# dkarpushkin/rs-pathtracing

Hardware: AMD Instinct MI355X
Metric: Msamples/sec cornell_box 1920x1080x256spp at 1/2/4/8 MI355X; RMS pixel delta (higher is better)
Workload: dtype f64; 1 GPU; cornell_box.json 1920x1080 256spp depth 8; config=c2, width=1920, height=1080, spp=256, depth=8, seed=1, parallelism=single GPU, wf_slots=2

## Files before the change

### rs-pathtracing_amd/csrc/pt_accel.cpp

```cpp
#include "pt_accel.hpp"

#include <algorithm>
#include <cmath>
#include <cstdlib>
#include <cstring>
#include <stdexcept>

namespace pt {

DBox shape_box(const HostShape &s) {
    double lo[3], hi[3];
    switch (s.type) {
    case RECTANGLE:
        lo[0] = s.x0; lo[1] = s.y0; lo[2] = -0.0001;
        hi[0] = s.x1; hi[1] = s.y1; hi[2] = 0.0001;
        break;
    case MARCH:
        if (s.func == 0) {
            lo[0] = -1.45; lo[1] = -(1.45 / 2.05); lo[2] = -1.45;
            hi[0] = 1.45; hi[1] = 1.45 / 2.05; hi[2] = 1.45;
        } else {
            const double r = std::fabs(s.fr);
            lo[0] = lo[1] = lo[2] = -r;
            hi[0] = hi[1] = hi[2] = r;
        }
        break;
    case TORUS: {
        const double a = s.radius + s.tube_radius;
        lo[0] = -a; lo[1] = -a; lo[2] = -s.tube_radius;
        hi[0] = a; hi[1] = a; hi[2] = s.tube_radius;
        break;
    }
    default:
        lo[0] = lo[1] = lo[2] = -1.0;
        hi[0] = hi[1] = hi[2] = 1.0;
    }
    DBox b;
    for (int k = 0; k < 3; k++) {
        b.lo[k] = INFINITY;
        b.hi[k] = -INFINITY;
    }
    for (int i = 0; i < 2; i++)
        for (int j = 0; j < 2; j++)
            for (int k = 0; k < 2; k++) {
                double p[3] = {i ? hi[0] : lo[0], j ? hi[1] : lo[1], k ? hi[2] : lo[2]};
                for (int r = 0; r < 3; r++) {
                    double v = p[0] * s.direct[r][0] + p[1] * s.direct[r][1] + p[2] * s.direct[r][2] + s.direct[r][3];
                    b.lo[r] = std::min(b.lo[r], v);
                    b.hi[r] = std::max(b.hi[r], v);
                }
            }
    double extent = 0;
    for (int r = 0; r < 3; r++)
        extent = std::max({extent, std::fabs(b.lo[r]), std::fabs(b.hi[r]), b.hi[r] - b.lo[r]});
    double pad = 1e-7 * extent + 1e-9;
    if (s.type == MARCH) pad += 2.0 * std::fabs(s.step);
    for (int r = 0; r < 3; r++) {
        b.lo[r] -= pad;
        b.hi[r] += pad;
    }
    return b;
}

namespace {

struct Builder {
    const std::vector<DBox> &boxes;
    Accel &out;
    int leaf_max = 1;
    struct TNode {
        DNode n;
        int axis, left, right;
    };
    std::vector<TNode> tree;

    void thread(int t, int oct, size_t base) {
        const size_t me = out.nodes.size();
        out.nodes.push_back(tree[t].n);
        if (tree[t].left >= 0) {
            const bool neg = (oct >> tree[t].axis) & 1;
            thread(neg ? tree[t].right : tree[t].left, oct, base);
            thread(neg ? tree[t].left : tree[t].right, oct, base);
        }
        out.nodes[me].skip = (int32_t)(out.nodes.size() - base);
    }

    int emit(std::vector<int32_t> &ids, size_t a, size_t b) {
        const int me = (int)tree.size();
        tree.push_back(TNode{DNode{}, 0, -1, -1});
        DNode n{};
        for (int k = 0; k < 3; k++) {
            n.lo[k] = INFINITY;
            n.hi[k] = -INFINITY;
        }
        double clo[3] = {INFINITY, INFINITY, INFINITY}, chi[3] = {-INFINITY, -INFINITY, -INFINITY};
        for (size_t i = a; i < b; i++) {
            const DBox &x = boxes[ids[i]];
            for (int k = 0; k < 3; k++) {
                n.lo[k] = std::min(n.lo[k], x.lo[k]);
                n.hi[k] = std::max(n.hi[k], x.hi[k]);
                double c = 0.5 * (x.lo[k] + x.hi[k]);
                clo[k] = std::min(clo[k], c);
                chi[k] = std::max(chi[k], c);
            }
        }
        if (b - a <= (size_t)leaf_max) {
            n.first = (int32_t)out.leaf.size();
            n.count = (int32_t)(b - a);
            for (size_t i = a; i < b; i++) out.leaf.push_back(ids[i]);
            tree[me].n = n;
            return me;
        }
        int axis = 0;
        for (int k = 1; k < 3; k++)
            if (chi[k] - clo[k] > chi[axis] - clo[axis]) axis = k;
        if (b - a > 2) {
            constexpr int NB = 32;
            auto area = [](const double *lo, const double *hi) {
                const double x = hi[0] - lo[0], y = hi[1] - lo[1], z = hi[2] - lo[2];
                return x * y + y * z + z * x;
            };
            double best = INFINITY;
            int bk = -1, bi = -1;
            for (int k = 0; k < 3; k++) {
                const double ext = chi[k] - clo[k];
                if (!(ext > 0.0)) continue;
                int cnt[NB] = {};
                double blo[NB][3], bhi[NB][3];
                for (int j = 0; j < NB; j++)
                    for (int r = 0; r < 3; r++) blo[j][r] = INFINITY, bhi[j][r] = -INFINITY;
                for (size_t i = a; i < b; i++) {
                    const DBox &x = boxes[ids[i]];
                    int j = (int)((0.5 * (x.lo[k] + x.hi[k]) - clo[k]) / ext * NB);
                    j = j < 0 ? 0 : (j >= NB ? NB - 1 : j);
                    cnt[j]++;
                    for (int r = 0; r < 3; r++) blo[j][r] = std::min(blo[j][r], x.lo[r]), bhi[j][r] = std::max(bhi[j][r], x.hi[r]);
                }
                double rlo[NB][3], rhi[NB][3];
                int rc[NB];
                for (int j = NB - 1; j >= 0; j--) {
                    for (int r = 0; r < 3; r++) {
                        rlo[j][r] = j + 1 < NB ? std::min(rlo[j + 1][r], blo[j][r]) : blo[j][r];
                        rhi[j][r] = j + 1 < NB ? std::max(rhi[j + 1][r], bhi[j][r]) : bhi[j][r];
                    }
                    rc[j] = (j + 1 < NB ? rc[j + 1] : 0) + cnt[j];
                }
                double llo[3] = {INFINITY, INFINITY, INFINITY}, lhi[3] = {-INFINITY, -INFINITY, -INFINITY};
                int lc = 0;
                for (int j = 0; j + 1 < NB; j++) {
                    lc += cnt[j];
                    for (int r = 0; r < 3; r++) llo[r] = std::min(llo[r], blo[j][r]), lhi[r] = std::max(lhi[r], bhi[j][r]);
                    if (lc == 0 || rc[j + 1] == 0) continue;
                    const double c = lc * area(llo, lhi) + rc[j + 1] * area(rlo[j + 1], rhi[j + 1]);
                    if (c < best) best = c, bk = k, bi = j;
                }
            }
            if (bk >= 0) {
                const double ext = chi[bk] - clo[bk];
                auto left = [&](int32_t id) {
                    const DBox &x = boxes[id];
                    int j = (int)((0.5 * (x.lo[bk] + x.hi[bk]) - clo[bk]) / ext * NB);
                    j = j < 0 ? 0 : (j >= NB ? NB - 1 : j);
                    return j <= bi;
                };
                const size_t m = (size_t)(std::stable_partition(ids.begin() + a, ids.begin() + b, left) - ids.begin());
                if (m > a && m < b) {
                    const int l = emit(ids, a, m);
                    const int r = emit(ids, m, b);
                    n.count = 0;
                    n.first = 0;
                    tree[me] = TNode{n, bk, l, r};
                    return me;
                }
            }
        }
        size_t mid = a + (b - a) / 2;
        std::nth_element(ids.begin() + a, ids.begin() + mid, ids.begin() + b, [&](int32_t x, int32_t y) {
            double cx = boxes[x].lo[axis] + boxes[x].hi[axis], cy = boxes[y].lo[axis] + boxes[y].hi[axis];
            return cx < cy || (cx == cy && x < y);
        });
        const int l = emit(ids, a, mid);
        const int r = emit(ids, mid, b);
        n.count = 0;
        n.first = 0;
        tree[me] = TNode{n, axis, l, r};
        return me;
    }
};

}

static bool make_grid(Accel &a) {
    double lo[3], hi[3];
    for (int k = 0; k < 3; k++) lo[k] = INFINITY, hi[k] = -INFINITY;
    for (const DNode &n : a.nodes)
        for (int k = 0; k < 3; k++) lo[k] = std::min(lo[k], n.lo[k]), hi[k] = std::max(hi[k], n.hi[k]);
    for (int k = 0; k < 3; k++) {
        if (!(std::isfinite(lo[k]) && std::isfinite(hi[k]) && std::isfinite(hi[k] - lo[k]))) return false;
        double step = std::ldexp(1.0, std::ilogb(std::max(hi[k] - lo[k], 1e-300) / 65535.0));
        for (int guard = 0;; guard++) {
            const double g0 = std::floor(lo[k] / step) * step;
            if (std::isfinite(g0) && std::ceil((hi[k] - g0) / step) <= 65535.0 && g0 <= lo[k]) {
                a.qg0[k] = g0;
                a.qgs[k] = step;
                break;
            }
            step *= 2.0;
            if (!std::isfinite(step) || guard > 64) return false;
        }
    }
    return true;
}
static double q_down(const Accel &a, double v, int k) {
    double q = std::floor((v - a.qg0[k]) / a.qgs[k]);
    while (q > 0 && a.qg0[k] + q * a.qgs[k] > v) q -= 1.0;
    return std::max(0.0, std::min(65535.0, q));
}
static double q_up(const Accel &a, double v, int k) {
    double q = std::ceil((v - a.qg0[k]) / a.qgs[k]);
    while (q < 65535.0 && a.qg0[k] + q * a.qgs[k] < v) q += 1.0;
    return std::max(0.0, std::min(65535.0, q));
}

void build_qnodes(Accel &a, const Scene &sc) {
    const size_t per_oct = a.nodes.size() / BVH_OCTANTS;
    if (!make_grid(a)) return;
    std::vector<DNodeQ> out;
    out.reserve(a.nodes.size());
    std::vector<int32_t> rec_of(a.leaf.size() + 1, -1);
    std::vector<DLeafRec> recs;
    for (size_t ni = 0; ni < per_oct; ni++) {
        const DNode &n = a.nodes[ni];
        if (n.count != 1 || !(a.cnodes[ni].first_count >> 31)) continue;
        const int id = a.leaf[n.first];
        const DShape d = to_device(sc.shapes[id]);
        DLeafRec l{};
        l.m[0] = d.inv[0], l.m[1] = d.inv[5], l.m[2] = d.inv[10];
        l.m[3] = d.inv[3], l.m[4] = d.inv[7], l.m[5] = d.inv[11];
        l.shape = id;
        l.axis = d.axis;
        rec_of[n.first] = (int32_t)recs.size();
        recs.push_back(l);
    }
    double bound = 0.0;
    for (int k = 0; k < 3; k++) bound = std::max(bound, std::fabs(a.qg0[k]));
    for (size_t ni = 0; ni < a.nodes.size(); ni++) {
        const DNode &n = a.nodes[ni];
        const int oct = (int)(ni / per_oct);
        DNodeQ c{};
        for (int k = 0; k < 3; k++) {
            const double ql = q_down(a, n.lo[k], k), qh = q_up(a, n.hi[k], k);
            if (a.qg0[k] + ql * a.qgs[k] > n.lo[k] || a.qg0[k] + qh * a.qgs[k] < n.hi[k]) return;
            bound = std::max({bound, std::fabs(a.qg0[k] + ql * a.qgs[k]), std::fabs(a.qg0[k] + qh * a.qgs[k])});
            const bool neg = (oct >> k) & 1;
            c.q[k] = (uint16_t)(neg ? qh : ql);
            c.q[3 + k] = (uint16_t)(neg ? ql : qh);
        }
        if (n.count == 0) {
            if (n.skip < 0) return;
            c.link = (uint32_t)n.skip;
        } else {
            if ((size_t)n.skip != ni % per_oct + 1 || n.count > 63) return;
            const uint32_t fc = a.cnodes[ni].first_count;
            const bool direct = fc >> 31;
            uint32_t first = fc & 0xffffffu;
            if (direct) {
                if (rec_of[n.first] < 0) return;
                first = (uint32_t)rec_of[n.first];
            }
            c.link = 1u << 31 | (direct ? 1u << 30 : 0u) | (uint32_t)n.count << 24 | first;
        }
        out.push_back(c);
    }
    a.qnodes.swap(out);
    a.qleaves.swap(recs);
    a.qbound = (float)bound;
    if ((double)a.qbound < bound) a.qbound = std::nextafter(a.qbound, INFINITY);
}

std::vector<DQGrid> pack_qnodes(const Accel &a) {
    if (a.qnodes.empty()) return {};
    const size_t ro = qleaf_offset(a.nodes_per_octant()), rb = a.qleaves.size() * sizeof(DLeafRec);
    std::vector<DQGrid> buf((ro + rb) / sizeof(DQGrid));
    for (int k = 0; k < 3; k++) buf[0].g0[k] = a.qg0[k], buf[0].gs[k] = a.qgs[k];
    buf[0].bound = a.qbound;
    std::memcpy(&buf[1], a.qnodes.data(), a.qnodes.size() * sizeof(DNodeQ));
    if (rb) std::memcpy((char *)buf.data() + ro, a.qleaves.data(), rb);
    return buf;
}

Accel build_accel(const Scene &sc, int json_shapes, int leaf_max) {
    Accel a;
    a.boxes.reserve(sc.shapes.size());
    for (auto &s : sc.shapes) a.boxes.push_back(shape_box(s));
    std::vector<int32_t> rest;
    bool small = json_shapes <= LIN_MAX;
    for (int32_t i = 0; i < (int32_t)sc.shapes.size(); i++) {
        if (sc.shapes[i].type == MARCH) a.march.push_back(i);
        else if ((small && i < json_shapes) || sc.shapes[i].type == TORUS) a.lin.push_back(i);
        else rest.push_back(i);
    }
    if (rest.size() > 64) {
        auto ext = [&](int32_t i) {
            const DBox &b = a.boxes[i];
            return std::max({b.hi[0] - b.lo[0], b.hi[1] - b.lo[1], b.hi[2] - b.lo[2]});
        };
        std::vector<double> e;
        e.reserve(rest.size());
        for (int32_t i : rest) e.push_back(ext(i));
        std::nth_element(e.begin(), e.begin() + e.size() / 2, e.end());
        const double big = 64.0 * e[e.size() / 2];
        std::vector<int32_t> keep;
        keep.reserve(rest.size());
        for (int32_t i : rest) {
            if (ext(i) > big && a.lin.size() < (size_t)LIN_MAX) a.lin.push_back(i);
            else keep.push_back(i);
        }
        rest.swap(keep);
    }
    if (!rest.empty()) {
        Builder b{a.boxes, a};
        b.leaf_max = std::max(1, std::min(16, leaf_max));
        const int root = b.emit(rest, 0, rest.size());
        a.nodes.reserve(b.tree.size() * BVH_OCTANTS);
        for (int oct = 0; oct < BVH_OCTANTS; oct++) b.thread(root, oct, a.nodes.size());
    }
    a.cnodes.reserve(a.nodes.size());
    const size_t per_oct = a.nodes.size() / BVH_OCTANTS;
    for (size_t ni = 0; ni < a.nodes.size(); ni++) {
        const DNode &n = a.nodes[ni];
        const int oct = per_oct ? (int)(ni / per_oct) : 0;
        if (n.first < 0 || n.first >= (1 << 24) || n.count < 0 || n.count > 255)
            throw std::runtime_error("BVH too large for the compact node form (leaf index >= 2^24)");
        DNodeC c{};
        for (int k = 0; k < 3; k++) {
            float lo = (float)n.lo[k], hi = (float)n.hi[k];
            if ((double)lo > n.lo[k]) lo = std::nextafter(lo, -INFINITY);
            if ((double)hi < n.hi[k]) hi = std::nextafter(hi, INFINITY);
            const bool neg = (oct >> k) & 1;
            c.nr[k] = neg ? hi : lo;
            c.fr[k] = neg ? lo : hi;
        }
        c.skip = n.skip;
        for (int k = 0; k < 3; k++) a.bvh_bound = std::max({a.bvh_bound, std::fabs(c.nr[k]), std::fabs(c.fr[k])});
        if (n.count == 1 && a.leaf[n.first] >= 0 && a.leaf[n.first] < (1 << 24))
            c.first_count = (uint32_t)a.leaf[n.first] | 1u << 24 | 1u << 31;
        else
            c.first_count = (uint32_t)n.first | (uint32_t)n.count << 24;
        a.cnodes.push_back(c);
    }
    if (per_oct >= (size_t)BIG_BVH_NODES) {
        build_qnodes(a, sc);
    }
    return a;
}

}
```

### rs-pathtracing_amd/csrc/pt_accel.hpp

```cpp
#pragma once
#include <array>
#include <cstdint>
#include <vector>

#include "pt_scene.hpp"
#include "pt_types.hpp"

namespace pt {

constexpr int BVH_OCTANTS = 8;
struct Accel {
    std::vector<DNode> nodes;
    std::vector<DNodeC> cnodes;
    int nodes_per_octant() const { return (int)(nodes.size() / BVH_OCTANTS); }
    std::vector<int32_t> leaf;
    std::vector<int32_t> lin;
    std::vector<int32_t> march;
    std::vector<DBox> boxes;
    float bvh_bound = 0.f;
    std::vector<DNodeQ> qnodes;
    std::vector<DLeafRec> qleaves;
    double qg0[3] = {0, 0, 0}, qgs[3] = {0, 0, 0};
    float qbound = 0.f;
};

constexpr int LIN_MAX = 32;

Accel build_accel(const Scene &sc, int json_shapes, int leaf_max = 1);
void build_qnodes(Accel &a, const Scene &sc);

std::vector<DQGrid> pack_qnodes(const Accel &a);
static_assert(sizeof(DLeafRec) % sizeof(DQGrid) == 0, "pack_qnodes sizes its buffer in DQGrid units");

static_assert(sizeof(dev::Scene) == 136, "a new dev::Scene field must be set by view_set_scene or view_set_accel");
inline void view_set_scene(dev::Scene &v, const Scene &sc, const DShape *shapes, const DMaterial *mats,
                           const DTexture *tex, const DPerlin *perlin, const DImage *images, const uint8_t *pixels) {
    v.shapes = shapes;
    v.mats = mats;
    v.tex = tex;
    v.perlin = perlin;
    v.images = images;
    v.pixels = pixels;
    v.nmats = (int)sc.materials.size();
    v.ext = scene_builds(sc).ext;
}
inline void view_set_accel(dev::Scene &v, const DNodeC *nodes, const DQGrid *qnodes, const int32_t *leaf,
                           const int32_t *lin, const int32_t *march, const DBox *boxes, int nnodes, int nlin,
                           int nmarch, float bvh_bound) {
    v.nodes = nodes;
    v.qnodes = qnodes;
    v.leaf = leaf;
    v.lin = lin;
    v.march = march;
    v.boxes = boxes;
    v.nnodes = nnodes;
    v.nlin = nlin;
    v.nmarch = nmarch;
    v.bvh_bound = bvh_bound;
}
inline void view_set_accel(dev::Scene &v, const Accel &a, const DNodeC *nodes, const DQGrid *qnodes,
                           const int32_t *leaf, const int32_t *lin, const int32_t *march, const DBox *boxes) {
    view_set_accel(v, nodes, qnodes, leaf, lin, march, boxes, a.nodes_per_octant(), (int)a.lin.size(),
                   (int)a.march.size(), a.bvh_bound);
}
inline void view_set_accel(dev::Scene &v, const dev::Scene &a) {
    view_set_accel(v, a.nodes, a.qnodes, a.leaf, a.lin, a.march, a.boxes, a.nnodes, a.nlin, a.nmarch, a.bvh_bound);
}
constexpr size_t VIEW_ACCEL_BUFS = 6;
inline std::array<const void *, 13> view_buffers(const dev::Scene &v) {
    return {v.nodes, v.qnodes, v.leaf,   v.lin,    v.march,  v.boxes, v.shapes,
            v.mats,  v.tex,    v.perlin, v.images, v.pixels, v.guard};
}
inline void view_of_host(dev::Scene &v, const Scene &sc, const Accel &a, const std::vector<DShape> &shapes,
                         const std::vector<DMaterial> &mats, const std::vector<DQGrid> &qbuf) {
    auto ptr = [](const auto &vec) { return vec.empty() ? nullptr : vec.data(); };
    view_set_scene(v, sc, ptr(shapes), ptr(mats), ptr(sc.textures), ptr(sc.perlins), ptr(sc.images), ptr(sc.pixels));
    view_set_accel(v, a, ptr(a.cnodes), ptr(qbuf), ptr(a.leaf), ptr(a.lin), ptr(a.march), ptr(a.boxes));
}

DBox shape_box(const HostShape &s);

}
```

### rs-pathtracing_amd/csrc/pt_device.hpp

```cpp
#pragma once
#include <hip/hip_runtime.h>

#include <cstdint>

#include "pt_lprof.hpp"
#include "pt_march.hpp"
#include "pt_torus.hpp"
#include "pt_types.hpp"

namespace pt {
namespace dev {

__device__ __forceinline__ bool stopped(const int *flag) {
    return flag && __hip_atomic_load(flag, __ATOMIC_RELAXED, __HIP_MEMORY_SCOPE_SYSTEM) != 0;
}

struct V3 {
    double x, y, z;
};
PT_HD V3 v3(double x, double y, double z) { return V3{x, y, z}; }
PT_HD V3 add(V3 a, V3 b) { return v3(a.x + b.x, a.y + b.y, a.z + b.z); }
PT_HD V3 sub(V3 a, V3 b) { return v3(a.x - b.x, a.y - b.y, a.z - b.z); }
PT_HD double dot(V3 a, V3 b) { return a.x * b.x + a.y * b.y + a.z * b.z; }
PT_HD V3 scale(V3 a, double s) { return v3(a.x * s, a.y * s, a.z * s); }
// ... 1 lines not shown
PT_HD V3 neg(V3 a) { return v3(-a.x, -a.y, -a.z); }
PT_HD V3 normalize(V3 a) { return divs(a, sqrt(dot(a, a))); }
PT_HD bool approx_zero(double a) { return fabs(a - 0.0) < 1e-15; }

constexpr uint64_t GAMMA = 0x9E3779B97F4A7C15ull;
PT_HD uint64_t mix64(uint64_t z) {
    z = (z ^ (z >> 30)) * 0xBF58476D1CE4E5B9ull;
    z = (z ^ (z >> 27)) * 0x94D049BB133111EBull;
    return z ^ (z >> 31);
}
PT_HD uint64_t sample_key(uint64_t seed, uint64_t pixel, uint64_t sample) {
    uint64_t k = mix64(seed ^ 0x6A09E667F3BCC909ull);
    k = mix64(k + (pixel + 1) * GAMMA);
    return mix64(k + (sample + 1) * 0xD1B54A32D192ED03ull);
}
PT_HD double bits_to_double(uint64_t b) {
    union {
        uint64_t u;
        double d;
    } x;
    x.u = b;
    return x.d;
}
struct Rng {
    uint64_t s;
    PT_HD uint64_t next() {
        s += GAMMA;
        return mix64(s);
    }
    PT_HD double gen() { return (double)(next() >> 11) * (1.0 / 9007199254740992.0); }
    PT_HD double uniform(double lo, double sc) {
        double v = bits_to_double((next() >> 12) | (1023ull << 52));
        return (v - 1.0) * sc + lo;
    }
};

PT_HD V3 xf_point(const double *m, V3 p) {
    return v3(p.x * m[0] + p.y * m[1] + p.z * m[2] + m[3], p.x * m[4] + p.y * m[5] + p.z * m[6] + m[7],
              p.x * m[8] + p.y * m[9] + p.z * m[10] + m[11]);
}
PT_HD V3 xf_vector(const double *m, V3 v) {
    return v3(v.x * m[0] + v.y * m[1] + v.z * m[2], v.x * m[4] + v.y * m[5] + v.z * m[6],
              v.x * m[8] + v.y * m[9] + v.z * m[10]);
}
PT_HD V3 xf_normal(const double *m, V3 n) {
    return v3(n.x * m[0] + n.y * m[4] + n.z * m[8], n.x * m[1] + n.y * m[5] + n.z * m[9],
              n.x * m[2] + n.y * m[6] + n.z * m[10]);
}



PT_HD bool sphere_t(V3 o, V3 d, double min_t, double max_t, double *t) {
    double a = dot(d, d);
    double hb = dot(d, o);
    double c = dot(o, o) - 1.0;
    double disc = hb * hb - a * c;
    if (disc < 0.0) return false;
    double x;
    if (disc == 0.0) {
        x = -hb * a;
    } else {
        double sq = sqrt(disc);
        x = (-hb - sq) / a;
        if (x < min_t || x > max_t) {
            x = (-hb + sq) / a;
            if (x < min_t || x > max_t) return false;
        }
    }
    *t = x;
    return true;
}
PT_HD bool axis_ray_ok(const V3 &o, const V3 &d) {
    const double sum = o.x + o.y + o.z + d.x + d.y + d.z;
    return sum - sum == 0.0 && fabs(d.x) > 1e-200 && fabs(d.y) > 1e-200 && fabs(d.z) > 1e-200;
}
PT_HD bool sphere_axis_t(const double *m, V3 ro, V3 rd, double min_t, double max_t, double *t) {
    const V3 o = v3(ro.x * m[0] + m[3], ro.y * m[5] + m[7], ro.z * m[10] + m[11]);
    const V3 d = v3(rd.x * m[0], rd.y * m[5], rd.z * m[10]);
    return sphere_t(o, d, min_t, max_t, t);
}
PT_HD bool rect_t(const double *p, V3 o, V3 d, double min_t, double max_t, double *t) {
    double tt = -o.z / d.z;
    if (tt < min_t || tt > max_t) return false;
    double px = o.x + d.x * tt, py = o.y + d.y * tt;
    if (px < p[0] || px > p[2] || py < p[1] || py > p[3]) return false;
    *t = tt;
    return true;
}
PT_HD bool cube_t(V3 o, V3 d, double min_t, double max_t, double *t) {
    double lx = (-1.0 - o.x) / d.x, ly = (-1.0 - o.y) / d.y, lz = (-1.0 - o.z) / d.z;
    double ux = (1.0 - o.x) / d.x, uy = (1.0 - o.y) / d.y, uz = (1.0 - o.z) / d.z;
    double tmin = fmax(fmax(fmax(fmin(lx, ux), fmin(ly, uy)), fmin(lz, uz)), min_t);
    double tmax = fmin(fmin(fmin(fmax(lx, ux), fmax(ly, uy)), fmax(lz, uz)), max_t);
    if (tmin > tmax || tmin > max_t) return false;
    *t = tmin;
    return true;
}

PT_HD V3 heart_gradient(V3 p) {
    double a = p.x * p.x + (9.0 / 4.0) * p.y * p.y + p.z * p.z - 1.0;
    a = 3.0 * a * a;
    double z2 = p.z * p.z;
    double z3 = z2 * p.z;
    return v3(2.0 * p.x * (a - z3), (9.0 / 2.0) * p.y * (a - 0.05 * z3),
              2.0 * p.z * (a - p.z * (1.5 * p.x * p.x + (27.0 / 40.0) * p.y * p.y)));
}

PT_HD march::FParams shape_params(const DShape &S) {
    march::FParams F;
    F.func = S.func;
    F.pad = 0;
    F.k[0] = S.fk[0];
    F.k[1] = S.fk[1];
    F.k[2] = S.fk[2];
    F.k[3] = S.fk[3];
    F.radius = S.fradius;
    return F;
}

struct Ray {
    V3 o, d;
};

PT_HD void note_guard(unsigned long long *guard) {
#if defined(__HIP_DEVICE_COMPILE__)
    if (guard) atomicAdd(guard, 1ull);
#else
    if (guard) ++*guard;
#endif
}

PT_HD void note_stop(unsigned long long *counters, bool worked) {
#if defined(__HIP_DEVICE_COMPILE__)
    if (!counters) return;
    atomicAdd(counters + 1, 1ull);
    if (worked) atomicAdd(counters + 2, 1ull);
#else
    (void)counters;
    (void)worked;
#endif
}

template <bool STATS, int FK = march::F_ANY, bool MARCHED = true, bool EXT = false>
PT_HD bool shape_test(const DShape &s, const Ray &r, double min_t, double max_t, double *t, Ctr *ct,
                      unsigned long long *guard = nullptr) {
    if (STATS) ct->c[s.type == TORUS ? C_TEST_TORUS : C_TEST_SPHERE + s.type]++;
    if (s.type == RECTANGLE) {
        const double *m = s.inv;
        const double oz = r.o.x * m[8] + r.o.y * m[9] + r.o.z * m[10] + m[11];
        const double dz = r.d.x * m[8] + r.d.y * m[9] + r.d.z * m[10];
        const double tt = -oz / dz;
        if (tt < min_t || tt > max_t) return false;
        PT_LP(RECT_ROWS);
        const double ox = r.o.x * m[0] + r.o.y * m[1] + r.o.z * m[2] + m[3];
        const double oy = r.o.x * m[4] + r.o.y * m[5] + r.o.z * m[6] + m[7];
        const double dx = r.d.x * m[0] + r.d.y * m[1] + r.d.z * m[2];
        const double dy = r.d.x * m[4] + r.d.y * m[5] + r.d.z * m[6];
        const double px = ox + dx * tt, py = oy + dy * tt;
        if (px < s.p[0] || px > s.p[2] || py < s.p[1] || py > s.p[3]) return false;
        *t = tt;
        return true;
    }
    V3 o = xf_point(s.inv, r.o);
    V3 d = xf_vector(s.inv, r.d);
    switch (s.type) {
    case SPHERE: return sphere_t(o, d, min_t, max_t, t);
    case RECTANGLE: return rect_t(s.p, o, d, min_t, max_t, t);
    case CUBE: return cube_t(o, d, min_t, max_t, t);
    case TORUS:
        if (!EXT) return false;
        return torus::torus_t(s.p[0], s.p[1], o.x, o.y, o.z, d.x, d.y, d.z, min_t, max_t, t);
    default: {
        if (!MARCHED) return false;
        march::MarchStats ms{0, 0, 0, 0};
        bool h = march::func_march<STATS, FK>(shape_params(s), s.p[0], s.depth, o.x, o.y, o.z, d.x, d.y, d.z, min_t, max_t,
                                          t, &ms);
        if (ms.guard) note_guard(guard);
        if (STATS) {
            ct->c[C_MARCH_STEPS] += ms.steps;
            ct->c[C_MARCH_BLOCKS] += ms.blocks;
            ct->c[C_MARCH_TRIES] += ms.tries;
            ct->c[C_MARCH_GUARD] += ms.guard;
        }
        return h;
    }
    }
}

template <class T>
PT_HD T uniform_load(const T *p) {
#if defined(__HIP_DEVICE_COMPILE__)
    return *(const __attribute__((address_space(4))) T *)p;
#else
    return *p;
#endif
}

PT_HD int uniform_index(int i) {
#if defined(__HIP_DEVICE_COMPILE__)
    return __builtin_amdgcn_readfirstlane(i);
#else
    return i;
#endif
}

PT_HD DShape uniform_shape(const DShape *p) {
    DShape s;
#pragma unroll
    for (int k = 0; k < 12; k++) s.inv[k] = uniform_load(&p->inv[k]);
#pragma unroll
    for (int k = 0; k < 4; k++) s.p[k] = uniform_load(&p->p[k]);
    s.type = uniform_load(&p->type);
    s.material = uniform_load(&p->material);
    s.depth = uniform_load(&p->depth);
    s.func = uniform_load(&p->func);
#pragma unroll
    for (int k = 0; k < 4; k++) s.fk[k] = uniform_load(&p->fk[k]);
    s.fradius = uniform_load(&p->fradius);
    return s;
}

PT_HD DBox uniform_box(const DBox *p) {
    DBox b;
#pragma unroll
    for (int k = 0; k < 3; k++) {
        b.lo[k] = uniform_load(&p->lo[k]);
        b.hi[k] = uniform_load(&p->hi[k]);
    }
    return b;
}

PT_HD uint32_t tile_position(uint32_t k, uint32_t tiles_x, uint32_t world) {
    if (world <= 1) return k;
    const uint32_t ty = k / tiles_x;
    return ty * tiles_x + (k % tiles_x + ty) % tiles_x;
}
PT_HD uint32_t tile_logical(uint32_t p, uint32_t tiles_x, uint32_t world) {
    if (world <= 1) return p;
    const uint32_t ty = p / tiles_x;
    return ty * tiles_x + (p % tiles_x + tiles_x - ty % tiles_x) % tiles_x;
}

PT_HD Ray load_ray(const double *rays, size_t i) {
    Ray r;
    r.o = v3(rays[i * 6 + 0], rays[i * 6 + 1], rays[i * 6 + 2]);
    r.d = v3(rays[i * 6 + 3], rays[i * 6 + 4], rays[i * 6 + 5]);
    return r;
}
PT_HD void store_rgb(double *out, size_t i, V3 c) {
    out[i * 3 + 0] = c.x;
    out[i * 3 + 1] = c.y;
    out[i * 3 + 2] = c.z;
}

PT_HD bool slab(const double *lo, const double *hi, const Ray &r, V3 inv, double min_t, double max_t) {
    double tx1 = (lo[0] - r.o.x) * inv.x, tx2 = (hi[0] - r.o.x) * inv.x;
    double ty1 = (lo[1] - r.o.y) * inv.y, ty2 = (hi[1] - r.o.y) * inv.y;
    double tz1 = (lo[2] - r.o.z) * inv.z, tz2 = (hi[2] - r.o.z) * inv.z;
    double tn = fmax(fmax(fmin(tx1, tx2), fmin(ty1, ty2)), fmax(fmin(tz1, tz2), min_t));
    double tf = fmin(fmin(fmax(tx1, tx2), fmax(ty1, ty2)), fmin(fmax(tz1, tz2), max_t));
    return tn <= tf;
}

PT_HD bool wave_all(bool p) {
#if defined(__HIP_DEVICE_COMPILE__)
    return __all(p);
#else
    return p;
#endif
}
PT_HD bool sphere_axis_rec(const double *m, V3 ro, V3 rd, double min_t, double max_t, double *t) {
    const V3 o = v3(ro.x * m[0] + m[3], ro.y * m[1] + m[4], ro.z * m[2] + m[5]);
    const V3 d = v3(rd.x * m[0], rd.y * m[1], rd.z * m[2]);
    return sphere_t(o, d, min_t, max_t, t);
}

template <bool STATS>
PT_HD void bvh_leaf_test(const Scene &sc, const Ray &r, bool axis_ok, int first, int count, bool direct,
                         double min_t, double &best, int &who, Ctr *ct) {
    for (int k = 0; k < count; k++) {
        int i = direct ? first : sc.leaf[first + k];
        PT_LP(BVH_LEAF);
        double t;
        const DShape &S = sc.shapes[i];
        bool h;
        if (axis_ok && S.axis) {
            if (STATS) ct->c[C_TEST_SPHERE]++;
            h = sphere_axis_t(S.inv, r.o, r.d, min_t, best, &t);
        } else {
            h = shape_test<STATS, march::F_ANY, false>(S, r, min_t, best, &t, ct);
        }
        if (h && (t < best || i > who)) {
            best = t;
            who = i;
        }
    }
}

template <bool STATS = false, bool EXT = false, bool FMA_SLAB = false, bool QN = false, int PART = 3>
PT_HD void closest_nomarch(const Scene &sc, const Ray &r, V3 inv, double min_t, double *best_t, int *who_out,
                           Ctr *ct = nullptr, bool any = false) {
    double best = *best_t;
    int who = *who_out;
    for (int k = 0; k < ((PART & 1) ? sc.nlin : 0); k++) {
        if (any && wave_all(who >= 0)) break;
        const int i = uniform_index(uniform_load(&sc.lin[k]));
        const DShape s = uniform_shape(&sc.shapes[i]);
        PT_LP(ULIST_SHAPE);
        if (s.type == CUBE || s.type == SPHERE) {
            if (STATS) ct->c[C_NODE_SLABS]++;
            const DBox b = uniform_box(&sc.boxes[i]);
            if (!slab(b.lo, b.hi, r, inv, min_t, best)) continue;
            PT_LP(UBOX_PASS);
        }
        double t;
        if (shape_test<STATS, march::F_ANY, false, EXT>(s, r, min_t, best, &t, ct) && (t < best || i > who)) {
            best = t;
            who = i;
        }
    }
    const int oct = (__builtin_signbit(r.d.x) ? 1 : 0) | (__builtin_signbit(r.d.y) ? 2 : 0) |
                    (__builtin_signbit(r.d.z) ? 4 : 0);
    const DNodeC *nodes = sc.nodes + (size_t)oct * (size_t)sc.nnodes;
    auto open_inf = [](double m) { return __builtin_isinf(m) ? __builtin_nan("") : m; };
    const double mx = FMA_SLAB ? open_inf(-(r.o.x * inv.x)) : 0.0, my = FMA_SLAB ? open_inf(-(r.o.y * inv.y)) : 0.0,
                 mz = FMA_SLAB ? open_inf(-(r.o.z * inv.z)) : 0.0;
    auto tx = [&](float b) { return FMA_SLAB ? __builtin_fma((double)b, inv.x, mx) : ((double)b - r.o.x) * inv.x; };
    auto ty = [&](float b) { return FMA_SLAB ? __builtin_fma((double)b, inv.y, my) : ((double)b - r.o.y) * inv.y; };
    auto tz = [&](float b) { return FMA_SLAB ? __builtin_fma((double)b, inv.z, mz) : ((double)b - r.o.z) * inv.z; };
    const bool axis_ok = FMA_SLAB && axis_ray_ok(r.o, r.d);
    constexpr bool S32 = FMA_SLAB;
    constexpr bool Q = S32 && QN;
    auto axis32 = [&](double o, double iv, float *i32, float *lo32, float *hi32) {
        const double m = -(o * iv);
        const bool fits = fabs(iv) < 1e30 && fabs(iv) > 1e-30 && fabs(m) < 1e30;
        const double e = (0x1p-21 * (1.0 + 0x1p-20)) * ((double)sc.bvh_bound + fabs(o)) * fabs(iv) + 1e-30;
        *i32 = (float)iv;
        *lo32 = fits ? (float)(m - e) : __builtin_nanf("");
        *hi32 = fits ? (float)(m + e) : __builtin_nanf("");
    };
    auto axisq = [&](int k, double o, double iv, float *si, float *gln, float *glf) {
        const double m = -(o * iv);
        const float i32 = (float)iv;
        const double s64 = (double)i32 * sc.qnodes->gs[k];
        const double e = 0x1p-19 * ((double)sc.qnodes->bound + fabs(o)) * fabs(iv) + 1e-30;
        const double g = sc.qnodes->g0[k] * (double)i32;
        const bool fits = fabs(iv) < 1e30 && fabs(iv) > 1e-30 && fabs(m) < 1e30 && fabs(s64) > 1e-30 &&
                          fabs(s64) < 1e30 && fabs(g) < 1e30;
        *si = (float)s64;
        *gln = fits ? (float)(g + (m - e)) : __builtin_nanf("");
        *glf = fits ? (float)(g + (m + e)) : __builtin_nanf("");
    };
    float ix = 0.f, iy = 0.f, iz = 0.f, lox = 0.f, loy = 0.f, loz = 0.f, hix = 0.f, hiy = 0.f, hiz = 0.f;
    if (Q) {
        axisq(0, r.o.x, inv.x, &ix, &lox, &hix);
        axisq(1, r.o.y, inv.y, &iy, &loy, &hiy);
        axisq(2, r.o.z, inv.z, &iz, &loz, &hiz);
    } else if (S32) {
        axis32(r.o.x, inv.x, &ix, &lox, &hix);
        axis32(r.o.y, inv.y, &iy, &loy, &hiy);
        axis32(r.o.z, inv.z, &iz, &loz, &hiz);
    }
    typedef float f2v __attribute__((ext_vector_type(2)));
    const f2v pa_i = {ix, iy}, pa_m = {lox, loy}, pb_i = {iz, ix}, pb_m = {loz, hix}, pc_i = {iy, iz},
              pc_m = {hiy, hiz};
    const float mt32 = S32 ? (float)(min_t - fabs(min_t) * 0x1p-20) : 0.f;
    float best32 = S32 ? (float)(best + fabs(best) * 0x1p-20) : 0.f;
    int n = any && who >= 0 ? sc.nnodes : (FMA_SLAB && sc.nnodes > 1 ? 1 : 0);
    if (!(PART & 2)) n = sc.nnodes;
    if (Q) {
        const DNodeQ *qn = (const DNodeQ *)(sc.qnodes + 1) + (size_t)oct * (size_t)sc.nnodes;
        while (n < sc.nnodes) {
            const uint4 raw = *(const uint4 *)(qn + n);
            PT_LP(BVH_NODE);
            if (STATS) ct->c[C_NODE_SLABS]++;
            const f2v a = __builtin_elementwise_fma((f2v){(float)(raw.x & 0xffffu), (float)(raw.x >> 16)}, pa_i, pa_m);
            const f2v b = __builtin_elementwise_fma((f2v){(float)(raw.y & 0xffffu), (float)(raw.y >> 16)}, pb_i, pb_m);
            const f2v c = __builtin_elementwise_fma((f2v){(float)(raw.z & 0xffffu), (float)(raw.z >> 16)}, pc_i, pc_m);
            const bool enter = fmaxf(fmaxf(a.x, a.y), fmaxf(b.x, mt32)) <= fminf(fminf(b.y, c.x), fminf(c.y, best32));
            const uint32_t link = raw.w;
            if (enter) {
                PT_LP(BVH_ENTER);
                if (link >> 31) {
                    const int first = (int)(link & 0xffffffu), count = (int)(link >> 24 & 0x3fu);
                    if ((link >> 30) & 1u) {
                        const DLeafRec &L = ((const DLeafRec *)((const char *)sc.qnodes + qleaf_offset(sc.nnodes)))[first];
                        const int i = L.shape;
                        double t;
                        bool h;
                        if (axis_ok && L.axis) {
                            if (STATS) ct->c[C_TEST_SPHERE]++;
                            h = sphere_axis_rec(L.m, r.o, r.d, min_t, best, &t);
                        } else {
                            h = shape_test<STATS, march::F_ANY, false>(sc.shapes[i], r, min_t, best, &t, ct);
                        }
                        if (h && (t < best || i > who)) {
                            best = t;
                            who = i;
                        }
                    } else {
                        bvh_leaf_test<STATS>(sc, r, axis_ok, first, count, (link >> 30) & 1u, min_t, best, who, ct);
                    }
                    best32 = (float)(best + fabs(best) * 0x1p-20);
                }
                n++;
            } else {
                n = (link >> 31) ? n + 1 : (int)link;
            }
        }
    }
    while (!Q && n < sc.nnodes) {
        const DNodeC nd = nodes[n];
        PT_LP(BVH_NODE);
        if (STATS) ct->c[C_NODE_SLABS]++;
        bool enter;
        if (S32) {
            const f2v a = __builtin_elementwise_fma((f2v){nd.nr[0], nd.nr[1]}, pa_i, pa_m);
            const f2v b = __builtin_elementwise_fma((f2v){nd.nr[2], nd.fr[0]}, pb_i, pb_m);
            const f2v c = __builtin_elementwise_fma((f2v){nd.fr[1], nd.fr[2]}, pc_i, pc_m);
            enter = fmaxf(fmaxf(a.x, a.y), fmaxf(b.x, mt32)) <= fminf(fminf(b.y, c.x), fminf(c.y, best32));
        } else {
            const double tn = fmax(fmax(tx(nd.nr[0]), ty(nd.nr[1])), fmax(tz(nd.nr[2]), min_t));
            const double tf = fmin(fmin(tx(nd.fr[0]), ty(nd.fr[1])), fmin(tz(nd.fr[2]), best));
            enter = tn <= tf;
        }
        if (enter) {
            PT_LP(BVH_ENTER);
            const int first = (int)(nd.first_count & 0xffffffu), count = (int)(nd.first_count >> 24 & 0x7fu);
            const bool direct = nd.first_count >> 31;
            bvh_leaf_test<STATS>(sc, r, axis_ok, first, count, direct, min_t, best, who, ct);
            if (S32) best32 = (float)(best + fabs(best) * 0x1p-20);
            n++;
        } else {
            n = nd.skip;
        }
    }
    *best_t = best;
    *who_out = who;
}

template <bool STATS = false, bool EXT = false>
PT_HD int closest(const Scene &sc, const Ray &r, double min_t, double max_t, double *best_t, Ctr *ct = nullptr) {
    double best = max_t;
    int who = -1;
    V3 inv = v3(1.0 / r.d.x, 1.0 / r.d.y, 1.0 / r.d.z);
    closest_nomarch<STATS, EXT>(sc, r, inv, min_t, &best, &who, ct);
    for (int k = 0; k < ((sc.diag & 1) ? 0 : sc.nmarch); k++) {
        int i = sc.march[k];
        const DBox &b = sc.boxes[i];
        if (STATS) ct->c[C_MARCH_SLABS]++;
        if (!slab(b.lo, b.hi, r, inv, min_t, best)) continue;
        double t;
        if (shape_test<STATS>(sc.shapes[i], r, min_t, best, &t, ct, sc.guard) && (t < best || i > who)) {
            best = t;
            who = i;
        }
    }
    *best_t = best;
    return who;
}

struct Hit {
    V3 p, n;
    bool front;
};
template <int FK = march::F_ANY>
PT_HD Hit finish(const DShape &s, const Ray &r, double t) {
    V3 o = xf_point(s.inv, r.o);
    V3 d = xf_vector(s.inv, r.d);
    V3 p = v3(o.x + d.x * t, o.y + d.y * t, o.z + d.z * t);
    V3 n;
    switch (s.type) {
    case SPHERE: n = s.inverse_normal ? neg(p) : p; break;
    case RECTANGLE: n = v3(0.0, 0.0, 1.0); break;
    case CUBE: {
        double ax = fabs(p.x), ay = fabs(p.y), az = fabs(p.z);
        double mc = fmax(fmax(ax, ay), az);
        if (mc == ax) n = v3(p.x, 0.0, 0.0);
        else if (mc == ay) n = v3(0.0, p.y, 0.0);
        else if (mc == az) n = v3(0.0, 0.0, p.z);
        else n = v3(__builtin_nan(""), __builtin_nan(""), __builtin_nan(""));
        break;
    }
    case TORUS:
        n = sub(p, scale(normalize(v3(p.x, p.y, 0.0)), s.p[0]));
        break;
    default: {
        double g[3];
        march::shape_gradient_k<FK>(shape_params(s), p.x, p.y, p.z, g);
        n = v3(g[0], g[1], g[2]);
        break;
    }
    }
    n = normalize(n);
    V3 wn = xf_normal(s.inv, n);
    Hit h;
    h.front = dot(wn, r.d) < 0.0;
    h.n = normalize(h.front ? wn : neg(wn));
    h.p = xf_point(s.dir, p);
    return h;
}

PT_HD void hit_uv(const DShape &s, const Ray &r, double t, double *u, double *v) {
    V3 o = xf_point(s.inv, r.o);
    V3 d = xf_vector(s.inv, r.d);
    V3 p = v3(o.x + d.x * t, o.y + d.y * t, o.z + d.z * t);
    const double PI = 3.141592653589793;
    switch (s.type) {
    case SPHERE: {
        const double theta = acos(-p.y);
        const double phi = atan2(-p.z, p.x) + PI;
        *u = phi / (2.0 * PI);
        *v = theta / PI;
        return;
    }
    case RECTANGLE:
        *u = (p.x - s.p[0]) / (s.p[2] - s.p[0]);
        *v = (p.y - s.p[1]) / (s.p[3] - s.p[1]);
        return;
    case CUBE: {
        double ax = fabs(p.x), ay = fabs(p.y), az = fabs(p.z);
        double mc = fmax(fmax(ax, ay), az);
        if (mc == ax) *u = p.y, *v = p.z;
        else if (mc == ay) *u = p.x, *v = p.z;
        else if (mc == az) *u = p.x, *v = p.y;
        else *u = *v = __builtin_nan("");
        return;
    }
    case TORUS: {
        const double theta = asin(p.z / s.p[1]);
        const double phi = acos(p.z / (s.p[0] + s.p[1] * cos(theta))) + PI;
        *u = phi / (2.0 * PI);
        *v = theta / PI;
        return;
    }
    default:
        if (s.func == march::F_DUPIN || s.func == march::F_HUNTS || s.func == march::F_CUSHION) *u = p.x, *v = p.y;
        else *u = *v = 0.0;
        return;
    }
}

PT_HD int32_t sat_i32(double x) {
    if (!(x == x)) return 0;
    if (x >= 2147483647.0) return 2147483647;
    if (x <= -2147483648.0) return -2147483647 - 1;
    return (int32_t)x;
}
PT_HD uint32_t sat_u32(double x) {
    if (!(x > 0.0)) return 0u;
    if (x >= 4294967295.0) return 4294967295u;
    return (uint32_t)x;
}

PT_HD double perlin_noise(const DPerlin &P, V3 p) {
    const double fx = floor(p.x), fy = floor(p.y), fz = floor(p.z);
    const uint32_t x = (uint32_t)sat_i32(fx), y = (uint32_t)sat_i32(fy), z = (uint32_t)sat_i32(fz);
    const double u = p.x - fx, v = p.y - fy, w = p.z - fz;
    const double u2 = u * u * (3.0 - 2.0 * u);
    const double v2 = v * v * (3.0 - 2.0 * v);
    const double w2 = w * w * (3.0 - 2.0 * w);
    double acc = 0.0;
    for (int c = 0; c < 8; c++) {
        const int d0 = c >> 2, d1 = (c >> 1) & 1, d2 = c & 1;
        const int32_t k = P.perm[0][(x + (uint32_t)d0) & 255u] ^ P.perm[1][(y + (uint32_t)d1) & 255u] ^
                          P.perm[2][(z + (uint32_t)d2) & 255u];
        const double fi = (double)d0, fj = (double)d1, fk = (double)d2;
        const double dot = P.ranvec[k][0] * (u - fi) + P.ranvec[k][1] * (v - fj) + P.ranvec[k][2] * (w - fk);
        acc = acc + (fi * u2 + (double)(1 - d0) * (1.0 - u2)) * (fj * v2 + (double)(1 - d1) * (1.0 - v2)) *
                        (fk * w2 + (double)(1 - d2) * (1.0 - w2)) * dot;
    }
    return acc;
}
PT_HD double perlin_turb(const DPerlin &P, V3 p) {
    const double n = perlin_noise(P, p);
    double acc = 0.0, weight = 1.0;
    for (int i = 0; i < 7; i++) {
        acc = acc + weight * n;
        weight *= 0.5;
    }
    return fabs(acc);
}

PT_HD V3 tex_value(const Scene &sc, int node, double u, double v, V3 p) {
    const double PI = 3.141592653589793;
    for (int guard = 0; guard < 64; guard++) {
        const DTexture &t = sc.tex[node];
        switch (t.type) {
        case TEX_SOLID: return v3(t.c[0], t.c[1], t.c[2]);
        case TEX_CHECKER: {
            const double sines = sin(t.c[0] * p.x) * sin(t.c[1] * p.y) * sin(t.c[2] * p.z);
            node = sines < 0.0 ? t.odd : t.even;
            break;
        }
        case TEX_UVCHECKER: {
            const double sines = sin(v * t.c[0] * PI) * sin(u * t.c[1] * PI);
            node = sines < 0.0 ? t.odd : t.even;
            break;
        }
        case TEX_NOISE: {
            const double s = 0.5 * (1.0 + sin(t.c[0] * p.z + 10.0 * perlin_turb(sc.perlin[t.aux], p)));
            return v3(1.0 * s, 1.0 * s, 1.0 * s);
        }
        default: {
            const DImage im = sc.images[t.aux];
            const double uc = u < 0.0 ? 0.0 : (u > 1.0 ? 1.0 : u);
            const double vc = 1.0 - (v < 0.0 ? 0.0 : (v > 1.0 ? 1.0 : v));
            uint32_t x = sat_u32(uc * (double)im.width), y = sat_u32(vc * (double)im.height);
            x = x < im.width ? x : im.width - 1;
            y = y < im.height ? y : im.height - 1;
            const uint8_t *px = sc.pixels + im.offset + ((size_t)y * im.width + x) * 4;
// ... 356 lines not shown
```

### rs-pathtracing_amd/csrc/pt_types.hpp

```cpp
#pragma once
#include <cstdint>

#include "pt_dims.hpp"

namespace pt {

enum ShapeKind : int32_t { SPHERE = 0, RECTANGLE = 1, CUBE = 2, MARCH = 3, TORUS = 4 };
enum MaterialKind : int32_t { LAMBERTIAN = 0, METAL = 1, DIELECTRIC = 2, DIFFUSE_LIGHT = 3, EMPTY = 4 };

struct alignas(64) DShape {
    int32_t type, material, inverse_normal, depth;
    double inv[12];
    int32_t func;
    int32_t axis;
    int32_t pad[2];
    double p[4];
    double dir[12];
    double fk[4];
    double fradius;
    double pad2[3];
};
static_assert(sizeof(DShape) == 320, "DShape is five cache lines");

struct alignas(8) DMaterial {
    int32_t type, tex;
    double albedo[3];
    double fuzz, ior;
    double emit[3];
};

enum TextureKind : int32_t { TEX_SOLID = 0, TEX_CHECKER = 1, TEX_UVCHECKER = 2, TEX_NOISE = 3, TEX_IMAGE = 4 };
struct alignas(8) DTexture {
    int32_t type, odd, even, aux;
    double c[3];
};
struct DPerlin {
    int32_t perm[3][256];
    double ranvec[256][3];
};
struct DImage {
    uint64_t offset;
    uint32_t width, height;
};

struct alignas(64) DNode {
    double lo[3], hi[3];
    int32_t skip, first, count, pad;
};
static_assert(sizeof(DNode) == 64, "DNode is one cache line");

struct alignas(32) DNodeC {
    float nr[3], fr[3];
    int32_t skip;
    uint32_t first_count;
};
static_assert(sizeof(DNodeC) == 32, "DNodeC is half a cache line");

struct alignas(16) DNodeQ {
    uint16_t q[6];
    uint32_t link;
};
static_assert(sizeof(DNodeQ) == 16, "DNodeQ is a quarter cache line");
__host__ __device__ inline size_t qleaf_offset(int nnodes_per_octant) {
    return 64 + ((size_t)(8 * (size_t)nnodes_per_octant + 1) * 16 + 63) / 64 * 64;
}
struct alignas(64) DQGrid {
    double g0[3], gs[3];
    float bound;
    float pad[3];
};
static_assert(sizeof(DQGrid) == 64, "DQGrid is one cache line");

struct alignas(64) DLeafRec {
    double m[6];
    int32_t shape, axis;
    int32_t pad[2];
};
static_assert(sizeof(DLeafRec) == 64, "DLeafRec is one 64-byte record");

struct DBox {
    double lo[3], hi[3];
};

struct FrameParams {
    double pos[3], right[3], up[3], left_top[3];
    double pixel_resolution;
    double s11;
    uint64_t seed;
    uint32_t width, height, spp, depth;
    uint32_t rank, world, tiles_x, tile_begin;
    uint32_t tile_count, compact;
    uint32_t s_begin, s_end;
    const int *stop;
};

enum Counter : int {
    C_SAMPLES, C_BOUNCES, C_TEST_SPHERE, C_TEST_RECT, C_TEST_CUBE, C_TEST_MARCH, C_NODE_SLABS, C_MARCH_SLABS,
    C_MARCH_STEPS, C_MARCH_TRIES, C_MARCH_BLOCKS, C_HITS, C_LAMBERT, C_METAL, C_DIELECTRIC, C_REJECT_TRIES,
    C_UNWIND, C_TEST_TORUS, C_MARCH_GUARD, C_COUNT
};
struct Ctr {
    uint64_t c[C_COUNT];
};

namespace dev {
struct Scene {
    const DShape *__restrict__ shapes;
    const DMaterial *__restrict__ mats;
    const DNodeC *__restrict__ nodes;
    const DQGrid *__restrict__ qnodes;
    const int32_t *__restrict__ leaf;
    const int32_t *__restrict__ lin;
    const int32_t *__restrict__ march;
    const DBox *__restrict__ boxes;
    const DTexture *__restrict__ tex;
    const DPerlin *__restrict__ perlin;
    const DImage *__restrict__ images;
    const uint8_t *__restrict__ pixels;
    int nnodes, nlin, nmarch, diag;
    int nmats;
    int ext;
    float bvh_bound;
    unsigned long long *guard;
};
}

constexpr double T_MIN = 0.001;

}
```

Baseline: 2201 Msamples/s.

## Group rectangles sharing a rotation to reuse transformed ray terms

At build time, the linear shape list is reordered so rectangles with identical 3x3 inverse rotation rows sit together, and later members are tagged with a grouped flag bit. In the device linear-list loop, rectangles get an inline intersection path that reuses the rotated ray origin and direction from the previous group member, recomputing only the translation terms. This aims to cut repeated f64 dot products for axis-aligned Cornell box walls, at the cost of a reordered list (tie-break by index is kept) and a flag bit taken from the shape index range.

```diff
diff --git a/rs-pathtracing_amd/csrc/pt_accel.cpp b/rs-pathtracing_amd/csrc/pt_accel.cpp
--- a/rs-pathtracing_amd/csrc/pt_accel.cpp
+++ b/rs-pathtracing_amd/csrc/pt_accel.cpp
@@ -289,6 +289,37 @@
     return buf;
 }
 
+void group_rectangles(std::vector<int32_t> &lin, const Scene &sc) {
+    constexpr int NW = 9;
+    auto row = [&](int32_t i, uint64_t (&w)[NW]) {
+        const DShape d = to_device(sc.shapes[i]);
+        bool ok = sc.shapes[i].type == RECTANGLE;
+        for (int k = 0; k < NW; k++) {
+            const double v = d.inv[4 * (k / 3) + k % 3];
+            std::memcpy(&w[k], &v, 8);
+            ok = ok && v == v;
+        }
+        return ok;
+    };
+    std::vector<int32_t> out;
+    std::vector<char> taken(lin.size(), 0);
+    out.reserve(lin.size());
+    for (size_t k = 0; k < lin.size(); k++) {
+        if (taken[k]) continue;
+        const int32_t i = lin[k] & LIN_ID_MASK;
+        out.push_back(i);
+        uint64_t w[NW], v[NW];
+        if (!row(i, w)) continue;
+        for (size_t j = k + 1; j < lin.size(); j++) {
+            const int32_t o = lin[j] & LIN_ID_MASK;
+            if (taken[j] || !row(o, v) || std::memcmp(w, v, sizeof w) != 0) continue;
+            taken[j] = 1;
+            out.push_back(o | LIN_GROUPED);
+        }
+    }
+    lin.swap(out);
+}
+
 Accel build_accel(const Scene &sc, int json_shapes, int leaf_max) {
     Accel a;
     a.boxes.reserve(sc.shapes.size());
@@ -318,6 +349,7 @@
         }
         rest.swap(keep);
     }
+    group_rectangles(a.lin, sc);
     if (!rest.empty()) {
         Builder b{a.boxes, a};
         b.leaf_max = std::max(1, std::min(16, leaf_max));
diff --git a/rs-pathtracing_amd/csrc/pt_accel.hpp b/rs-pathtracing_amd/csrc/pt_accel.hpp
--- a/rs-pathtracing_amd/csrc/pt_accel.hpp
+++ b/rs-pathtracing_amd/csrc/pt_accel.hpp
@@ -27,6 +27,7 @@
 constexpr int LIN_MAX = 32;
 
 Accel build_accel(const Scene &sc, int json_shapes, int leaf_max = 1);
+void group_rectangles(std::vector<int32_t> &lin, const Scene &sc);
 void build_qnodes(Accel &a, const Scene &sc);
 
 std::vector<DQGrid> pack_qnodes(const Accel &a);
diff --git a/rs-pathtracing_amd/csrc/pt_device.hpp b/rs-pathtracing_amd/csrc/pt_device.hpp
--- a/rs-pathtracing_amd/csrc/pt_device.hpp
+++ b/rs-pathtracing_amd/csrc/pt_device.hpp
@@ -327,11 +327,38 @@
                            Ctr *ct = nullptr, bool any = false) {
     double best = *best_t;
     int who = *who_out;
+    double g_pz = 0.0, g_dz = 1.0, g_ox = 0.0, g_oy = 0.0, g_dx = 0.0, g_dy = 0.0;
     for (int k = 0; k < ((PART & 1) ? sc.nlin : 0); k++) {
         if (any && wave_all(who >= 0)) break;
-        const int i = uniform_index(uniform_load(&sc.lin[k]));
+        const int entry = uniform_index(uniform_load(&sc.lin[k]));
+        const int i = entry & LIN_ID_MASK;
         const DShape s = uniform_shape(&sc.shapes[i]);
         PT_LP(ULIST_SHAPE);
+        if (s.type == RECTANGLE) {
+            if (STATS) ct->c[C_TEST_RECT]++;
+            const double *m = s.inv;
+            if (!(entry & LIN_GROUPED)) {
+                g_pz = r.o.x * m[8] + r.o.y * m[9] + r.o.z * m[10];
+                g_dz = r.d.x * m[8] + r.d.y * m[9] + r.d.z * m[10];
+                g_ox = r.o.x * m[0] + r.o.y * m[1] + r.o.z * m[2];
+                g_oy = r.o.x * m[4] + r.o.y * m[5] + r.o.z * m[6];
+                g_dx = r.d.x * m[0] + r.d.y * m[1] + r.d.z * m[2];
+                g_dy = r.d.x * m[4] + r.d.y * m[5] + r.d.z * m[6];
+            }
+            const double oz = g_pz + m[11];
+            const double tt = -oz / g_dz;
+            bool h = !(tt < min_t || tt > best);
+            if (h) {
+                PT_LP(RECT_ROWS);
+                const double px = (g_ox + m[3]) + g_dx * tt, py = (g_oy + m[7]) + g_dy * tt;
+                h = !(px < s.p[0] || px > s.p[2] || py < s.p[1] || py > s.p[3]);
+            }
+            if (h && (tt < best || i > who)) {
+                best = tt;
+                who = i;
+            }
+            continue;
+        }
         if (s.type == CUBE || s.type == SPHERE) {
             if (STATS) ct->c[C_NODE_SLABS]++;
             const DBox b = uniform_box(&sc.boxes[i]);
diff --git a/rs-pathtracing_amd/csrc/pt_types.hpp b/rs-pathtracing_amd/csrc/pt_types.hpp
--- a/rs-pathtracing_amd/csrc/pt_types.hpp
+++ b/rs-pathtracing_amd/csrc/pt_types.hpp
@@ -125,6 +125,9 @@
 };
 }
 
+constexpr int32_t LIN_GROUPED = 1 << 30;
+constexpr int32_t LIN_ID_MASK = LIN_GROUPED - 1;
+
 constexpr double T_MIN = 0.001;
 
 }
```

Result: faster. 2236 Msamples/s, median of 6 (+1.6%).
